# BarisYazici/deep-rl-grasping

Measured on NVIDIA H100. Metric: SAC grad-steps/sec (batch 256, 64x64 depth), higher is better.
Workload: dtype bf16x3 (fp32-faithful split, f32 accumulate)

## Files before the change

### deep-rl-grasping_b200/csrc/common.cuh

```cuda
#pragma once
#include <cuda_runtime.h>
#include <stdint.h>

#include <string>
#include <vector>

namespace b2g {

#ifdef __CUDACC__
__device__ __forceinline__ void pdl_wait() { asm volatile("griddepcontrol.wait;" ::: "memory"); }
__device__ __forceinline__ void pdl_trigger() { asm volatile("griddepcontrol.launch_dependents;" ::: "memory"); }
template <typename... KArgs, typename... Args>
inline cudaError_t launch_pdl(void (*kernel)(KArgs...), dim3 grid, dim3 block, size_t smem, cudaStream_t s, bool pdl, Args... args) {
  cudaLaunchConfig_t cfg{};
  cfg.gridDim = grid; cfg.blockDim = block; cfg.dynamicSmemBytes = smem; cfg.stream = s;
  cudaLaunchAttribute attr[1];
  attr[0].id = cudaLaunchAttributeProgrammaticStreamSerialization;
  attr[0].val.programmaticStreamSerializationAllowed = 1;
  cfg.attrs = attr; cfg.numAttrs = pdl ? 1 : 0;
  return cudaLaunchKernelEx(&cfg, kernel, KArgs(args)...);
}
#endif
bool pdl_enabled();

// ... 76 lines not shown
struct TailArgs {
  int B, H, A, feat_dim;
  float gamma, target_entropy;
  int grad_scale_B;
  const float* z0_pi; const float* z0_vf; const float* z0_q1; const float* z0_q2; const float* z0_vt;
  int z0v_ld;
  HeadW pi, vf, q1, q2, vt;
  const float* ksig; const float* bsig;
  HeadG g_pi, g_vf, g_q1, g_q2;
  float* g_ksig; float* g_bsig;
  const float* log_alpha; float* g_log_alpha;
  const float* act;  int act_stride;
  const float* eps;
  const float* rew; const float* done;
  float* a0_pi; float* a0_vf; float* a0_q1; float* a0_q2;
  float* dz1_pi; float* dz1_vf; float* dz1_q1; float* dz1_q2;
  float* dz0_pi;
  float* dz0_v3;
  uint16_t* dz0_pi_p[2]; uint16_t* dz0_v3_p[2];
  float* per_sample;
  float* pi_out;
  float* metrics;
};
cudaError_t tail_launch(const TailArgs& a, cudaStream_t s);

struct HeadsWgradArgs {
  const float* X0[4];
  const float* dz0[4];
  const float* a0[4];
  const float* dz1[4];
  float* g_k0[4]; float* g_b0[4]; float* g_k1[4]; float* g_b1[4];
  int M0[4];
  int dz0_ld[4];
  int x0_ld, B;
  int H;
};
void heads_wgrad_launch(const HeadsWgradArgs& a, cudaStream_t s);
cudaError_t act_launch(const TailArgs& t, int n, int deterministic, float* act_out, cudaStream_t s);

enum Metric : int {
  MET_POLICY_LOSS = 0, MET_QF1_LOSS, MET_QF2_LOSS, MET_VALUE_LOSS, MET_ENT_COEF_LOSS, MET_ENTROPY,
  MET_MEAN_Q1, MET_MEAN_Q2, MET_MEAN_V, MET_MEAN_LOGP, MET_GN_PI, MET_GN_VALUES, MET_COUNT = 16
};

struct OptimArgs {
  float* P; float* Mo; float* Vo; const float* G;
  float* T;
// ... 129 lines not shown
```

### deep-rl-grasping_b200/csrc/engine_v2.cu

```cuda
#include <cuda_bf16.h>

#include <algorithm>
#include <cstdio>
#include <cstdlib>
#include <cstring>

#include "sac_internal.cuh"

namespace b2g {
namespace {

struct Gather2Args {
  GatherArgs g;
  uint16_t* s1[2][3];
  uint16_t* fp[3][3];
  int KF;
};

__device__ __forceinline__ void split3(float y, uint16_t& p0, uint16_t& p1, uint16_t& p2) {
  const __nv_bfloat16 h0 = __float2bfloat16_rn(y);
  const float r1 = y - __bfloat162float(h0);
  const __nv_bfloat16 h1 = __float2bfloat16_rn(r1);
  const float r2 = r1 - __bfloat162float(h1);
  p0 = __bfloat16_as_ushort(h0); p1 = __bfloat16_as_ushort(h1); p2 = __bfloat16_as_ushort(__float2bfloat16_rn(r2));
// ... 98 lines not shown
      split3(av, p0, p1, p2);
      const size_t po = (size_t)b * a.KF + feat_dim + tid;
      a.fp[1][0][po] = p0; a.fp[1][1][po] = p1; a.fp[1][2][po] = p2;
    }
    if (tid == 32) {
      float r = g.rew[slot];
      if (g.normc[4] != 0.0) r = (float)fmin(fmax((double)r * g.normc[0], -g.normc[2]), g.normc[2]);
      g.rew_out[b] = r;
      g.done_out[b] = g.done[slot];
    }
  }
}

struct Plane2Job {
  const float* src;
  uint16_t* dst[3];
  int R, N, np;
  int transpose;
  int ld, off0;
  int k1_ci;
  int tile_start;
};

__global__ void __launch_bounds__(256) planes2_kernel(const Plane2Job* __restrict__ jobs, const int* __restrict__ cta_job) {
  __shared__ float tile[64][33];
  const Plane2Job job = jobs[cta_job[blockIdx.x]];
  const int t = blockIdx.x - job.tile_start;
  const int tiles_n = (job.N + 31) / 32;
  const int r0 = (t / tiles_n) * 64, n0 = (t % tiles_n) * 32;
  const int tid = threadIdx.x;
  const bool vec_ok = (job.N & 3) == 0;
  for (int i = tid; i < 64 * 8; i += 256) {
    const int rr = i >> 3, c4 = i & 7, r = r0 + rr, n = n0 + 4 * c4;
    float4 v = make_float4(0.f, 0.f, 0.f, 0.f);
    if (r < job.R) {
      const float* sp = job.src + (size_t)r * job.N + n;
      if (vec_ok && n + 3 < job.N) v = *reinterpret_cast<const float4*>(sp);
      else { if (n < job.N) v.x = sp[0]; if (n + 1 < job.N) v.y = sp[1]; if (n + 2 < job.N) v.z = sp[2]; if (n + 3 < job.N) v.w = sp[3]; }
    }
    tile[rr][4 * c4] = v.x; tile[rr][4 * c4 + 1] = v.y; tile[rr][4 * c4 + 2] = v.z; tile[rr][4 * c4 + 3] = v.w;
    if (!job.transpose && r < job.R) {
      const float x[4] = {v.x, v.y, v.z, v.w};
      uint16_t p[3][4];
#pragma unroll
      for (int u = 0; u < 4; ++u) split3(x[u], p[0][u], p[1][u], p[2][u]);
      for (int k = 0; k < job.np; ++k) {
        uint16_t* d = job.dst[k] + (size_t)r * job.ld + job.off0 + n;
        if (n + 3 < job.N && (((size_t)r * job.ld + job.off0 + n) & 3) == 0)
          *reinterpret_cast<uint2*>(d) = make_uint2((uint32_t)p[k][0] | ((uint32_t)p[k][1] << 16), (uint32_t)p[k][2] | ((uint32_t)p[k][3] << 16));
        else
          for (int u = 0; u < 4; ++u) if (n + u < job.N) d[u] = p[k][u];
      }
    }
  }
  if (!job.transpose) return;
  __syncthreads();
  {
    const int nn = tid >> 3, g8 = tid & 7, n = n0 + nn, rb = r0 + 8 * g8;
    if (n < job.N && rb < job.R) {
      uint16_t p[3][8];
#pragma unroll
      for (int u = 0; u < 8; ++u) split3(tile[8 * g8 + u][nn], p[0][u], p[1][u], p[2][u]);
      const size_t o = (size_t)(n + job.off0) * job.ld + rb;
      for (int k = 0; k < job.np; ++k) {
        uint16_t* d = job.dst[k] + o;
        if (job.k1_ci) {
          for (int u = 0; u < 8; ++u) if (rb + u < job.R) d[conv1_krow(rb + u, job.k1_ci) - rb] = p[k][u];
        } else if (rb + 7 < job.R && (o & 7) == 0)
          *reinterpret_cast<uint4*>(d) = make_uint4((uint32_t)p[k][0] | ((uint32_t)p[k][1] << 16), (uint32_t)p[k][2] | ((uint32_t)p[k][3] << 16),
                                                    (uint32_t)p[k][4] | ((uint32_t)p[k][5] << 16), (uint32_t)p[k][6] | ((uint32_t)p[k][7] << 16));
        else
          for (int u = 0; u < 8; ++u) if (rb + u < job.R) d[u] = p[k][u];
      }
    }
  }
}

int add_maps(V2State& v, uint16_t* const* planes, int np, int rank, std::initializer_list<uint64_t> dims, std::initializer_list<uint64_t> strides_b,
             std::initializer_list<uint32_t> box, std::initializer_list<uint32_t> estr = {}, bool allow_whole = true, int swizzle = 128) {
  uint64_t d[5] = {1, 1, 1, 1, 1}, s[5] = {0, 0, 0, 0, 0};
  uint32_t bx[5] = {1, 1, 1, 1, 1}, es[5] = {1, 1, 1, 1, 1};
  int i = 0; for (auto x : dims) d[i++] = x;
  i = 0; for (auto x : strides_b) s[i++] = x;
  i = 0; for (auto x : box) bx[i++] = x;
  i = 0; for (auto x : estr) es[i++] = x;
  if (rank >= 5 || np < 1) return -1;
  size_t rows = 1;
// ... 175 lines not shown
  if (int rc = palloc(v.W1T[0], 3, (size_t)64 * K1)) return rc;
  if (int rc = palloc(v.W1T[1], 3, (size_t)32 * K1)) return rc;
  for (int n = 0; n < 3; ++n) {
    if (int rc = palloc(v.W2T[n], 3, 64 * 512)) return rc;
    if (int rc = palloc(v.W3T[n], 3, 64 * 576)) return rc;
    if (int rc = palloc(v.WfT[n], 3, 512 * 1024)) return rc;
    if (int rc = palloc(v.K0T[n], 3, (size_t)(n == 1 ? 3 : 1) * h->H * KF)) return rc;
  }
  return 0;
}

int v2_create(b2g_sac* h) {
  V2State& v = h->v2;
  g_mk_state = &v;
  const int B = h->B, Ci = h->Cimg, Cp = s2d_channels(Ci), K1 = 64 * Cp, KF = v.KF, FS = h->FS, H = h->H;
  const size_t n1 = (size_t)B * 225 * 32;
  const char* nets[3] = {"model/pi", "model/values_fn", "target/values_fn"};
  std::vector<Plane2Job> jobs;
  int start = 0;
  auto add_job = [&](const float* src, int R, int N, uint16_t* const* dst, int np, int transpose, int ld, int off0) {
    Plane2Job j{};
    j.src = src; j.R = R; j.N = N; j.np = np; j.transpose = transpose; j.ld = ld; j.off0 = off0; j.tile_start = start;
    for (int k = 0; k < np; ++k) j.dst[k] = dst[k];
    start += ((R + 63) / 64) * ((N + 31) / 32);
    jobs.push_back(j);
  };
  add_job(h->p("model/pi/cnn1/w"), 64 * Ci, 32, v.W1T[0], 3, 1, K1, 0);
  jobs.back().k1_ci = Ci;
  add_job(h->p("model/values_fn/cnn1/w"), 64 * Ci, 32, v.W1T[0], 3, 1, K1, 32);
  jobs.back().k1_ci = Ci;
  add_job(h->p("target/values_fn/cnn1/w"), 64 * Ci, 32, v.W1T[1], 3, 1, K1, 0);
  jobs.back().k1_ci = Ci;
  for (int n = 0; n < 3; ++n) {
    add_job(h->p(std::string(nets[n]) + "/cnn2/w"), 512, 64, v.W2T[n], 3, 1, 512, 0);
    add_job(h->p(std::string(nets[n]) + "/cnn3/w"), 576, 64, v.W3T[n], 3, 1, 576, 0);
    add_job(h->p(std::string(nets[n]) + "/cnn_fc1/w"), 1024, 512, v.WfT[n], 3, 1, 1024, 0);
  }
  add_job(h->p("model/pi/fc0/kernel"), h->feat_dim, H, v.K0T[0], 3, 1, KF, 0);
  add_job(h->p("model/values_fn/vf/fc0/kernel"), h->feat_dim, H, v.K0T[1], 3, 1, KF, 0);
  add_job(h->p("model/values_fn/qf1/fc0/kernel"), h->feat_dim + h->A, H, v.K0T[1], 3, 1, KF, H);
  add_job(h->p("model/values_fn/qf2/fc0/kernel"), h->feat_dim + h->A, H, v.K0T[1], 3, 1, KF, 2 * H);
  add_job(h->p("target/values_fn/vf/fc0/kernel"), h->feat_dim, H, v.K0T[2], 3, 1, KF, 0);
  for (int n = 0; n < 2; ++n) {
    add_job(h->p(std::string(nets[n]) + "/cnn2/w"), 512, 64, v.W2n[n], 2, 0, 64, 0);
    add_job(h->p(std::string(nets[n]) + "/cnn3/w"), 576, 64, v.W3n[n], 2, 0, 64, 0);
    add_job(h->p(std::string(nets[n]) + "/cnn_fc1/w"), 1024, 512, v.Wfn[n], 2, 0, 512, 0);
  }
  add_job(h->p("model/pi/fc0/kernel"), h->feat_dim, H, v.K0n[0], 2, 0, H, 0);
  add_job(h->p("model/values_fn/vf/fc0/kernel"), h->feat_dim, H, v.K0n[1], 2, 0, 3 * H, 0);
  add_job(h->p("model/values_fn/qf1/fc0/kernel"), h->feat_dim + h->A, H, v.K0n[1], 2, 0, 3 * H, H);
  add_job(h->p("model/values_fn/qf2/fc0/kernel"), h->feat_dim + h->A, H, v.K0n[1], 2, 0, 3 * H, 2 * H);
  v.n_plane_jobs = (int)jobs.size();
  v.plane_ctas = start;
  Plane2Job* dj = nullptr;
  if (int rc = dev_alloc(h->allocs, h->stream, &dj, jobs.size())) return rc;
  CK(cudaMemcpyAsync(dj, jobs.data(), jobs.size() * sizeof(Plane2Job), cudaMemcpyHostToDevice, h->stream));
  CK(cudaStreamSynchronize(h->stream));
  v.plane_jobs = dj;
  {
    std::vector<int> cj((size_t)start);
    for (size_t k = 0; k < jobs.size(); ++k)
      for (int t = jobs[k].tile_start; t < (k + 1 < jobs.size() ? jobs[k + 1].tile_start : start); ++t) cj[t] = (int)k;
    if (int rc = upload_table(h->allocs, h->stream, cj, &v.plane_cta_job)) return rc;
  }

// ... 355 lines not shown
    std::vector<const CgGroup*> pa(parts.begin(), parts.begin() + 2), pb(parts.begin() + 2, parts.end());
    std::vector<Wire> wa, wb;
    for (int n = 0; n < 2; ++n) {
      wa.push_back({1, 2 * n, 0, n, 128, 128, 0});
      wa.push_back({1, 2 * n + 1, 0, n, 64, 128, 1});
      wb.push_back({1, n, 0, 2 * n, 72, 108, 0});
      wb.push_back({2, n, 0, 2 * n, 144, 108, 1});
    }
    wb.push_back({2, 2, 1, 0, 1, 8, 1});
    wb.push_back({2, 2, 1, 1, 1, 8, 1});
    if (int rc = fuse_groups(h, pa, wa, "bwd_fused_fc", v.bwd_fused, n_ctr)) return rc;
    if (int rc = fuse_groups(h, pb, wb, "bwd_fused_conv", v.bwd_fused, n_ctr)) return rc;
  }
  if (int rc = dev_alloc(h->allocs, h->stream, &v.dep_ctr, (size_t)n_ctr)) return rc;
  v.n_dep_ctr = n_ctr;
  bind_counters(v.fwd_fused, v.dep_ctr);
  bind_counters(v.bwd_fused, v.dep_ctr);
  if (int rc = dev_alloc(h->allocs, h->stream, &v.d_maps, v.maps.size())) return rc;
  CK(cudaMemcpyAsync(v.d_maps, v.maps.data(), v.maps.size() * sizeof(CUtensorMap), cudaMemcpyHostToDevice, h->stream));
  CK(cudaStreamSynchronize(h->stream));
  return 0;
}

int v2_planes(b2g_sac* h, cudaStream_t s) {
  V2State& v = h->v2;
  planes2_kernel<<<v.plane_ctas, 256, 0, s>>>((const Plane2Job*)v.plane_jobs, v.plane_cta_job);
  return 0;
}

int v2_gather(b2g_sac* h, const GatherArgs& ga, cudaStream_t s) {
  V2State& v = h->v2;
  Gather2Args a{};
  a.g = ga;
  for (int w = 0; w < 2; ++w)
    for (int p = 0; p < 3; ++p) a.s1[w][p] = v.S[w][p];
  for (int n = 0; n < 3; ++n) for (int p = 0; p < 3; ++p) a.fp[n][p] = v.F[n][p];
  a.KF = v.KF;
  const dim3 grid(ga.B, ga.next_obs || ga.next_frame ? 2 : 1);
  switch (h->Cimg) {
    case 1: gather2_kernel<1><<<grid, 512, 0, s>>>(a); break;
    case 2: gather2_kernel<2><<<grid, 512, 0, s>>>(a); break;
    case 3: gather2_kernel<3><<<grid, 512, 0, s>>>(a); break;
    default: gather2_kernel<4><<<grid, 512, 0, s>>>(a); break;
  }
  return 0;
}

extern long long* g_cg_trace;
static long long* s_trace_buf = nullptr;
// ... 38 lines not shown
```

### deep-rl-grasping_b200/csrc/sac.cu

```cuda
#include <cuda_runtime.h>
#include <math.h>
#include <stdio.h>
#include <string.h>

#include <algorithm>
#include <chrono>
#include <map>
#include <tuple>
#include <string>
#include <vector>

#include "../../include/b200grasp.h"
#include "common.cuh"
#include "sac_internal.cuh"
#include "state.cuh"

using namespace b2g;

namespace b2g {
bool pdl_enabled() {
  static int v = -1;
  if (v < 0) { const char* e = getenv("B2G_PDL"); v = (e && e[0] == '0') ? 0 : 1; }
  return v != 0;
}
// ... 602 lines not shown
  cudaStream_t s = h->stream;
  int n = 0;
  int n_copy = 0;
  (void)n_copy;
  auto mark = [&](const char* name) {
    if (prof && prof->on) {
      cudaEvent_t e;
      cudaEventCreate(&e);
      cudaEventRecord(e, s);
      prof->ev.push_back(e);
      prof->names.push_back(name);
    }
  };
  mark("begin");
  PrepArgs pa = make_prep(h, h->cfg.seed + 0x9E3779B97F4A7C15ull * (unsigned long long)h->cfg.rank, sampled, apply);
  const bool fork = h->fork_leaves && !(prof && prof->on);
  cudaStream_t ax = fork ? h->aux : s;
  GatherArgs ga = make_gather(h, sampled, true);
  if (fork) {
    pa.defer_bump = 1; pa.skip_indices = 1;
    if (sampled) { ga.indices = nullptr; ga.rng_counters = h->counters; ga.seed = pa.seed; ga.indices_out = h->indices; }
    CK(cudaEventRecord(h->ev_aux[0], s));
    CK(cudaStreamWaitEvent(ax, h->ev_aux[0], 0));
    if (h->use_planes && !h->v2.on) { planes_launch(h->d_jobs, h->n_jobs, h->job_tiles, ax); ++n; }
    if (h->v2.on) { if (int rc = v2_planes(h, ax)) return rc; ++n; }
    CK(cudaMemsetAsync(h->z0[0], 0, (size_t)5 * h->B * h->H * sizeof(float), ax)); ++n_copy;
    if (h->v2.on) { CK(cudaMemsetAsync(h->v2.z0v, 0, (size_t)3 * h->B * h->H * sizeof(float), ax)); ++n_copy; }
    CK(cudaEventRecord(h->ev_aux[1], ax));
    prep_launch(pa, ax); ++n;
    CK(cudaMemsetAsync(h->G, 0, (size_t)(h->n_train + MET_COUNT) * sizeof(float), ax)); ++n_copy;
    CK(cudaEventRecord(h->ev_aux[6], ax));
  } else {
    prep_launch(pa, s); ++n; mark("prep");
  }
  if (h->v2.on) {
    if (!fork) { if (int rc = v2_planes(h, s)) return rc; ++n; mark("weight_planes_v2"); }
    if (int rc = v2_gather(h, ga, s)) return rc;
  } else gather_launch(ga, s);
  ++n; mark("gather_normalize");
  if (h->record_after_gather) CK(cudaEventRecord(h->record_after_gather, s));
  if (fork) CK(cudaStreamWaitEvent(s, h->ev_aux[1], 0));
  else {
    CK(cudaMemsetAsync(h->G, 0, (size_t)(h->n_train + MET_COUNT) * sizeof(float), s)); ++n_copy;
    CK(cudaMemsetAsync(h->z0[0], 0, (size_t)5 * h->B * h->H * sizeof(float), s)); ++n_copy;
    if (h->v2.on) { CK(cudaMemsetAsync(h->v2.z0v, 0, (size_t)3 * h->B * h->H * sizeof(float), s)); ++n_copy; }
    mark("zero_grads");
  }
  const int x3 = h->cfg.precision == B2G_PREC_BF16X3 ? 1 : 0;
  auto run_group = [&](GemmGroup& g, cudaStream_t s) -> int {
    if (g.tc) CK(gg_tc_launch(g.host.data(), (int)g.host.size(), g.total_tiles, g.host[0].flags, x3, h->num_sms, s));
    else gg_simt_launch(g.dev, (int)g.host.size(), g.total_tiles, s);
    ++n; mark(g.name.c_str());
    return 0;
  };
  if (h->v2.on) {
    CK(cudaMemsetAsync(h->v2.dep_ctr, 0, (size_t)h->v2.n_dep_ctr * sizeof(int), s)); ++n_copy;
    if (int rc = v2_launch(h, h->v2.fwd_fused[0], s)) return rc;
    ++n; mark("fwd_fused");
  } else {
    for (auto& g : h->fwd_groups) if (int rc = run_group(g, s)) return rc;
  }
  if (fork) CK(cudaStreamWaitEvent(s, h->ev_aux[6], 0));
  CK(tail_launch(make_tail(h, want_per_sample), s)); ++n; mark("heads_tail");
  auto make_optim = [&]() {
    OptimArgs oa{};
    oa.P = h->P; oa.Mo = h->Mo; oa.Vo = h->Vo; oa.G = h->G; oa.T = h->P + h->n_train;
    oa.n_pi = (int)h->n_pi; oa.n_values = (int)h->n_values; oa.n_ent = (int)h->n_ent; oa.n_target = (int)h->n_target;
    oa.step_consts = h->step_consts; oa.tau = h->cfg.tau; oa.grad_scale = 1.0f / (float)h->cfg.nranks;
    oa.metrics = h->metrics; oa.apply = apply ? 1 : 0;
    return oa;
  };
  const bool overlap = h->overlap_ar && h->cfg.nranks > 1 && !(h->dp_p2p && apply);
  const int64_t pi_fc1 = h->tensors[h->tindex.at("model/pi/" + std::string(h->cnn ? "cnn_fc1/w" : "fc0/kernel"))].off;
  const int64_t v_fc1 = h->tensors[h->tindex.at("model/values_fn/" + std::string(h->cnn ? "cnn_fc1/w" : "vf/fc0/kernel"))].off;
  auto nccl_ck = [&](int rc) -> int {
    if (rc != 0) return b2g_fail(B2G_ENCCL, std::string("nccl: ") + (g_nccl.GetErrorString ? g_nccl.GetErrorString(rc) : "?"));
    return 0;
  };
  bool dp_early_opt = false;
  if (h->v2.on) {
    h->v2.sm_reserve = 0;
    cudaStream_t lx = fork ? ax : s;
    if (fork) { CK(cudaEventRecord(h->ev_aux[2], s)); CK(cudaStreamWaitEvent(ax, h->ev_aux[2], 0)); }
    HeadsWgradArgs wa{};
    const char* hp[4] = {"model/pi", "model/values_fn/vf", "model/values_fn/qf1", "model/values_fn/qf2"};
    for (int q = 0; q < 4; ++q) {
      wa.X0[q] = h->F[q == 0 ? 0 : 1];
      wa.dz0[q] = q == 0 ? h->dz0_pi : h->dz0_v3 + (q - 1) * h->H;
      wa.dz0_ld[q] = q == 0 ? h->H : 3 * h->H;
      wa.a0[q] = h->a0[q]; wa.dz1[q] = h->dz1[q];
      wa.M0[q] = q >= 2 ? h->feat_dim + h->A : h->feat_dim;
      wa.g_k0[q] = h->g(std::string(hp[q]) + "/fc0/kernel"); wa.g_b0[q] = h->g(std::string(hp[q]) + "/fc0/bias");
      wa.g_k1[q] = h->g(std::string(hp[q]) + "/fc1/kernel"); wa.g_b1[q] = h->g(std::string(hp[q]) + "/fc1/bias");
    }
    wa.x0_ld = h->FS; wa.B = h->B; wa.H = h->H;
    heads_wgrad_launch(wa, lx); ++n; if (!fork) mark("heads_wgrad");
    if (!overlap) {
      if (int rc = v2_launch(h, h->v2.bwd_fused[0], s)) return rc;
      ++n; mark("bwd_fused");
    } else {
      if (int rc = v2_launch(h, h->v2.bwd_fused[1], s)) return rc;
      ++n; mark("bwd_fused_fc");
      CK(cudaMemcpyAsync(h->G + h->n_train, h->metrics, MET_GN_PI * sizeof(float), cudaMemcpyDeviceToDevice, s)); ++n_copy;
      CK(cudaEventRecord(h->ev_fork, s));
      CK(cudaStreamWaitEvent(h->side, h->ev_fork, 0));
      if (fork) { CK(cudaEventRecord(h->ev_aux[4], ax)); CK(cudaStreamWaitEvent(h->side, h->ev_aux[4], 0)); }
// ... 307 lines not shown
          }
      };
      patch(h->v2.bwd_fused);
      if (found && (t.off & 3) == 0) { h->dp_skip[k][0] = (int)(t.off >> 2); h->dp_skip[k][1] = (int)((t.off + 1024 * 512) >> 2); }
    }
  }
  h->dp_p2p = true;
  if (h->graph_exec) { cudaGraphExecDestroy(h->graph_exec); h->graph_exec = nullptr; }
  for (auto& g : h->pipe_graph) if (g) { cudaGraphExecDestroy(g); g = nullptr; }
  return 0;
}

int b2g_sac_destroy(b2g_sac* h) {
  if (!h) return 0;
  cudaSetDevice(h->cfg.device);
  if (h->stream) cudaStreamSynchronize(h->stream);
  if (h->graph_exec) cudaGraphExecDestroy(h->graph_exec);
  for (auto& g : h->pipe_graph) if (g) cudaGraphExecDestroy(g);
  for (void* q : h->dp_opened) cudaIpcCloseMemHandle(q);
  nccl_comm_destroy(h->nccl_comm2);
  nccl_comm_destroy(h->nccl_comm);
  if (h->side) cudaStreamDestroy(h->side);
  if (h->aux) { cudaStreamSynchronize(h->aux); cudaStreamDestroy(h->aux); }
  for (auto& e : h->ev_aux) if (e) cudaEventDestroy(e);
  if (h->ev_fork) cudaEventDestroy(h->ev_fork);
  if (h->ev_join) cudaEventDestroy(h->ev_join);
  for (void* q : h->allocs) cudaFree(q);
  for (int q = 0; q < 2; ++q) { if (h->hc_obs[q]) cudaFreeHost(h->hc_obs[q]); if (h->hc_next[q]) cudaFreeHost(h->hc_next[q]); }
  if (h->h_met) cudaFreeHost(h->h_met);
  if (h->h_cnt) cudaFreeHost(h->h_cnt);
  if (h->h_plan) cudaFreeHost(h->h_plan);
  if (h->h_rc) cudaFreeHost(h->h_rc);
  for (int k = 0; k < 2; ++k) { if (h->hp_stats[k]) cudaFreeHost(h->hp_stats[k]); if (h->ev_stats[k]) cudaEventDestroy(h->ev_stats[k]); }
  for (int j = 0; j < 2; ++j) {
    if (h->ev_h2d[j]) cudaEventDestroy(h->ev_h2d[j]);
    if (h->ev_consumed[j]) cudaEventDestroy(h->ev_consumed[j]);
    if (h->ev_met[j]) cudaEventDestroy(h->ev_met[j]);
    if (h->pm_met[j]) cudaFreeHost(h->pm_met[j]);
    if (h->pm_cnt[j]) cudaFreeHost(h->pm_cnt[j]);
  }
  if (h->cstream) cudaStreamDestroy(h->cstream);
  if (h->ev0) cudaEventDestroy(h->ev0);
  if (h->ev1) cudaEventDestroy(h->ev1);
  if (h->stream) cudaStreamDestroy(h->stream);
  delete h;
  return 0;
// ... 134 lines not shown
  DA(h->z0[0], 5 * B * h->H);
  for (int q = 1; q < 5; ++q) h->z0[q] = h->z0[0] + (size_t)q * B * h->H;
  for (int q = 0; q < 4; ++q) { DA(h->a0[q], B * h->H); DA(h->dz1[q], B * h->H); }
  DA(h->dz0_pi, B * h->H); DA(h->dz0_v3, B * 3 * h->H);
  DA(h->per_sample, 7 * B); DA(h->pi_out, B * h->A); DA(h->eps, B * h->A + 4); DA(h->rew_n, B); DA(h->done_n, B);
  DA(h->indices, B + 4);
#undef DA
  if (cudaMallocHost((void**)&h->h_met, (MET_COUNT + 2) * sizeof(float)) != cudaSuccess ||
      cudaMallocHost((void**)&h->h_cnt, 8 * sizeof(long long)) != cudaSuccess)
    return bail(b2g_fail(B2G_ECUDA, "cudaMallocHost failed"));
  for (int j = 0; j < 2; ++j) {
    if ((rc = dev_alloc(h->allocs, h->stream, &h->ps_obs[j], (size_t)B * h->Ec)) || (rc = dev_alloc(h->allocs, h->stream, &h->ps_next[j], (size_t)B * h->Ec))) return bail(rc);
    if (cudaEventCreateWithFlags(&h->ev_h2d[j], cudaEventDisableTiming) != cudaSuccess ||
        cudaEventCreateWithFlags(&h->ev_consumed[j], cudaEventDisableTiming) != cudaSuccess ||
        cudaEventCreateWithFlags(&h->ev_met[j], cudaEventDisableTiming) != cudaSuccess ||
        cudaMallocHost((void**)&h->pm_met[j], (MET_COUNT + 2) * sizeof(float)) != cudaSuccess ||
        cudaMallocHost((void**)&h->pm_cnt[j], 8 * sizeof(long long)) != cudaSuccess)
      return bail(b2g_fail(B2G_ECUDA, "pipelined-path resources"));
  }
  if (cudaStreamCreateWithFlags(&h->cstream, cudaStreamNonBlocking) != cudaSuccess) return bail(b2g_fail(B2G_ECUDA, "copy stream"));
  {
    const char* fk = getenv("B2G_FORK");
    if (!(fk && atoi(fk) == 0)) {
      if (cudaStreamCreateWithFlags(&h->aux, cudaStreamNonBlocking) != cudaSuccess) return bail(b2g_fail(B2G_ECUDA, "aux stream"));
      for (auto& e : h->ev_aux)
        if (cudaEventCreateWithFlags(&e, cudaEventDisableTiming) != cudaSuccess) return bail(b2g_fail(B2G_ECUDA, "aux events"));
      h->fork_leaves = true;
    }
  }
  {
    std::vector<double> ones(h->Ec, 1.0);
    if (cudaMemcpyAsync(h->d_istd, ones.data(), h->Ec * sizeof(double), cudaMemcpyHostToDevice, h->stream) != cudaSuccess ||
        cudaStreamSynchronize(h->stream) != cudaSuccess)
      return bail(b2g_fail(B2G_ECUDA, "init copy failed"));
  }
  if ((rc = build_groups(h))) return bail(rc);
  if (h->v2.on && (rc = v2_create(h))) return bail(rc);
  if (cfg->nranks > 1) {
    if (!cfg->nccl_id) return bail(b2g_fail(B2G_EINVAL, "nranks > 1 needs nccl_id"));
    if ((rc = nccl_comm_init(&h->nccl_comm, cfg->nranks, cfg->nccl_id, cfg->rank, cfg->nccl_lib))) return bail(rc);
    {
      const char* ov = getenv("B2G_AR_OVERLAP");
      const bool want_ov = h->v2.on && !(ov && ov[0] == '0');
      if (want_ov && g_nccl.CommSplit && g_nccl.GroupStart && g_nccl.GroupEnd) {
        if (g_nccl.CommSplit(h->nccl_comm, 0, cfg->rank, &h->nccl_comm2, nullptr) == 0 && h->nccl_comm2 &&
            cudaStreamCreateWithFlags(&h->side, cudaStreamNonBlocking) == cudaSuccess &&
            cudaEventCreateWithFlags(&h->ev_fork, cudaEventDisableTiming) == cudaSuccess &&
// ... 535 lines not shown
  s[4].pieces = {dev_piece(h->r_nfr, cap * sizeof(int))};
  s[5].pieces = {dev_piece(h->r_act, cap * h->A * sizeof(float))};
  s[6].pieces = {dev_piece(h->r_rew, cap * sizeof(float))};
  s[7].pieces = {dev_piece(h->r_done, cap * sizeof(float))};
  s[8].pieces = frame_pieces(h, lo, hi);
  for (int i = 0; i < 9; ++i) s[i].tag = kSacTags[i + 2];
  return s;
}

}

extern "C" {

int b2g_sac_state_save(b2g_sac* h, const char* path) {
  if (!h || !path) return b2g_fail(B2G_EINVAL, "NULL argument");
  B2G_USABLE(h);
  if (h->cfg.nranks > 1)
    return b2g_fail(B2G_ESTATE, "training-state files of data-parallel learners (nranks > 1) are not built: each rank holds only its "
                                "slice of the Adam moments");
  if (h->pipe_pending)
    return b2g_fail(B2G_ESTATE, "a host-pipelined step is in flight: call b2g_sac_pipeline_flush first (its losses would be lost)");
  CK(cudaSetDevice(h->cfg.device));
  CK(cudaStreamSynchronize(h->stream));
  if (h->aux) CK(cudaStreamSynchronize(h->aux));
  long long cnt[8];
  CK(cudaMemcpy(cnt, h->counters, sizeof cnt, cudaMemcpyDeviceToHost));
  SacHostState hs;
  hs.r_size = h->r_size; hs.head_seq = h->head_seq; hs.tail_seq = h->tail_seq; hs.next_fid = h->next_fid; hs.evicted = h->evicted;
  hs.lw.assign(h->lw.begin(), h->lw.end());
  hs.prev_next = h->prev_next;
  std::vector<int64_t> hv = {hs.r_size, hs.head_seq, hs.tail_seq, hs.next_fid, hs.evicted, (int64_t)hs.lw.size(), (int64_t)hs.prev_next.size()};
  for (const auto& q : hs.lw) { hv.push_back(q.first); hv.push_back(q.second); }
  hv.insert(hv.end(), hs.prev_next.begin(), hs.prev_next.end());
  std::vector<StateSection> secs(2);
  secs[0].tag = kSacTags[0]; secs[0].pieces = {host_piece(hv.data(), hv.size() * sizeof(int64_t))};
  secs[1].tag = kSacTags[1]; secs[1].pieces = {host_piece(cnt, sizeof cnt)};
  for (auto& s : sac_device_sections(h, hs.frame_lo(h->frame_cap), hs.next_fid)) secs.push_back(std::move(s));
  if (h->rms_mean) {
    StateSection r;
    r.tag = kRmsTag;
    r.pieces = {host_piece(&h->rms_count, sizeof(double)), dev_piece(h->rms_mean, h->E * sizeof(double)),
                dev_piece(h->rms_var, h->E * sizeof(double))};
    secs.push_back(std::move(r));
  }
  return state_write(path, STATE_KIND_SAC, sac_fingerprint_rms(h), secs);
}

// ... 24 lines not shown
  const int64_t cap = h->cfg.buffer_capacity, FC = h->frame_cap;
  if (rd.bytes(0) % 8 || rd.bytes(0) < 7 * 8 || rd.bytes(0) > (uint64_t)(7 + 2 * cap + 4 * FC) * 8)
    return b2g_fail(B2G_EINVAL, "corrupt replay bookkeeping in the training-state file");
  std::vector<int64_t> hv(rd.bytes(0) / 8);
  if (int rc = rd.read_host(0, hv.data(), hv.size() * 8)) return rc;
  SacHostState hs;
  hs.r_size = hv[0]; hs.head_seq = hv[1]; hs.tail_seq = hv[2]; hs.next_fid = hv[3]; hs.evicted = hv[4];
  const int64_t n_lw = hv[5], n_prev = hv[6];
  if (n_lw < 0 || n_prev < 0 || (int64_t)hv.size() != 7 + 2 * n_lw + n_prev || hs.r_size != hs.head_seq - hs.tail_seq || hs.r_size < 0 ||
      hs.r_size > cap || hs.tail_seq < 0 || hs.next_fid < 0 || hs.evicted < 0)
    return b2g_fail(B2G_EINVAL, "corrupt replay bookkeeping in the training-state file");
  for (int64_t i = 0; i < n_lw; ++i) hs.lw.emplace_back(hv[7 + 2 * i], hv[8 + 2 * i]);
  hs.prev_next.assign(hv.begin() + 7 + 2 * n_lw, hv.end());
  const int64_t lo = hs.frame_lo(FC);
  if (lo < 0 || lo > hs.next_fid || hs.next_fid - lo > FC) return b2g_fail(B2G_EINVAL, "corrupt replay bookkeeping in the training-state file");
  std::vector<StateSection> dev = sac_device_sections(h, lo, hs.next_fid);
  for (int i = 0; i < (int)dev.size(); ++i)
    if (rd.bytes(i + 2) != dev[i].bytes())
      return b2g_fail(B2G_EINVAL, "training-state section lengths do not match this handle's configuration");
  long long cnt[8];
  if (rd.bytes(1) != sizeof cnt) return b2g_fail(B2G_EINVAL, "training-state section lengths do not match this handle's configuration");
  if (int rc = rd.read_host(1, cnt, sizeof cnt)) return rc;
  CK(cudaStreamSynchronize(h->stream));
  if (h->aux) CK(cudaStreamSynchronize(h->aux));
  h->broken = true;
  for (int i = 0; i < (int)dev.size(); ++i)
    if (int rc = rd.read_pieces(i + 2, dev[i].pieces)) return rc;
  if (h->rms_mean) {
    double count = 0.0;
    if (int rc = rd.read_pieces(n_sec, {host_piece(&count, sizeof(double)), dev_piece(h->rms_mean, h->E * sizeof(double)),
                                        dev_piece(h->rms_var, h->E * sizeof(double))})) return rc;
    h->rms_count = count;
    obs_rms_derive(h);
  }
  h->ob_n = 0;
  CK(cudaMemcpy(h->counters, cnt, sizeof cnt, cudaMemcpyHostToDevice));
  h->r_size = hs.r_size; h->head_seq = hs.head_seq; h->tail_seq = hs.tail_seq; h->next_fid = hs.next_fid; h->evicted = hs.evicted;
  h->lw.assign(hs.lw.begin(), hs.lw.end());
  h->prev_next = hs.prev_next;
  h->planes_dirty = true;
  h->broken = false;
  return 0;
}

}
```

### deep-rl-grasping_b200/csrc/sac_internal.cuh

```cuda
#pragma once
#include <cuda_runtime.h>

#include <deque>
#include <map>
#include <string>
#include <tuple>
#include <vector>

#include "../../include/b200grasp.h"
#include "cg.cuh"
#include "common.cuh"
#include "host.cuh"

namespace b2g {
struct Tensor {
  std::string name;
  int ndim;
  int64_t shape[4];
  int64_t numel;
  int64_t off;
  int group;
};


// ... 7 lines not shown
  int KF = 576;
  uint16_t* S[2][3]{};
  uint16_t* H1[3][3]{};
  uint16_t* H2[3][3]{};
  uint16_t* H3[3][3]{};
  uint16_t* F[3][3]{};
  uint16_t* dz0pi[2]{};
  uint16_t* dz0v[2]{};
  uint16_t* dZ4[2][2]{};
  uint16_t* dZ3[2][2]{};
  uint16_t* dZ2[2][2]{};
  uint16_t* dZ1[2]{};
  uint16_t* W1T[2][3]{};
  uint16_t* W2T[3][3]{};
  uint16_t* W3T[3][3]{};
  uint16_t* WfT[3][3]{};
  uint16_t* K0T[3][3]{};
  uint16_t* W2n[2][2]{};
  uint16_t* W3n[2][2]{};
  uint16_t* Wfn[2][2]{};
  uint16_t* K0n[2][2]{};
  float* z0v = nullptr;
  void* plane_jobs = nullptr; int n_plane_jobs = 0, plane_ctas = 0;
  const int* plane_cta_job = nullptr;
  int sm_reserve = 0;
  std::vector<CUtensorMap> maps;
  std::vector<char> map_whole;
  std::vector<int> map_box_bytes;
  CUtensorMap* d_maps = nullptr;
  std::vector<CgGroup> fwd, bwd_groups;
  std::vector<CgGroup> fwd_fused, bwd_fused;
  int split_fc1 = 3;
  int split_fc1_dgrad = 1;
  int* dep_ctr = nullptr; int n_dep_ctr = 0;
  std::vector<int*> tabs;
  int dbg = 0;
};

}

struct b2g_sac;
namespace b2g {
int v2_alloc(b2g_sac* h);
int v2_create(b2g_sac* h);
int v2_planes(b2g_sac* h, cudaStream_t s);
int v2_gather(b2g_sac* h, const GatherArgs& ga, cudaStream_t s);
int v2_launch(b2g_sac* h, const CgGroup& g, cudaStream_t s);
int sac_act_rows(b2g_sac* h, const float* rows, int chunk, int deterministic);
int sac_replay_add_linked(b2g_sac* h, const float* c_obs, const float* c_next, const int64_t* obs_fid, const float* act,
                          const float* rew, const float* done, int n, int64_t* next_fid);
void obs_rms_derive(b2g_sac* h);
}

using namespace b2g;

struct b2g_sac {
  b2g_sac_cfg cfg{};
  bool cnn = false;
  int num_sms = 132;
  int B = 0, A = 0, H = 0, E = 0, Cimg = 0, feat_dim = 0, FS = 0;
  int Hi = 0, Wi = 0, H1 = 0, W1 = 0, H2 = 0, W2 = 0, H3 = 0, W3 = 0;
  std::vector<Tensor> tensors;
  std::map<std::string, int> tindex;
  int64_t n_pi = 0, n_values = 0, n_ent = 0, n_target = 0, n_train = 0, n_all = 0;
  float *P = nullptr, *Mo = nullptr, *Vo = nullptr, *G = nullptr;
  float* metrics = nullptr;
  cudaStream_t stream = nullptr;
  std::vector<void*> allocs;
// ... 43 lines not shown
  long long* pm_cnt[2]{};
  long long pipe_k = 0;
  bool pipe_pending = false;
  cudaEvent_t record_after_gather = nullptr;
  long long* counters = nullptr;
  double* step_consts = nullptr;
  float* d_lr = nullptr;
  float cur_lr = -1.f;
  std::vector<GemmGroup> fwd_groups, bwd_groups, act_groups;
  cudaGraphExec_t graph_exec = nullptr;
  bool use_graph = true;
  void* nccl_comm = nullptr;
  void* nccl_comm2 = nullptr;
  bool pipe_serial = false; int pipe_tune = 0; double pipe_t0 = 0, pipe_period[2] = {0, 0};
  bool dp_p2p = false;
  int* dp_x = nullptr;
  int* dp_sync = nullptr;
  float* dp_recv = nullptr;
  float* dp_P[8]{}; float* dp_G[8]{}; int* dp_X[8]{};
  std::vector<void*> dp_opened;
  int dp_skip[2][2]{};
  cudaStream_t side = nullptr;
  cudaStream_t aux = nullptr;
  cudaEvent_t ev_aux[7]{};
  bool fork_leaves = false;
  std::map<std::tuple<const void*, const void*, const void*, int>, int> col_ids;
  cudaEvent_t ev_fork = nullptr, ev_join = nullptr;
  bool overlap_ar = false;
  int ar_sms = 8;
  ColsumJob* d_colsum_early = nullptr;
  int n_colsum_early = 0, colsum_early_ctas = 0;
  cudaEvent_t ev0 = nullptr, ev1 = nullptr;
  float last_ms = 0.f;
  int launches = 0;
  std::vector<std::string> prof_names;
  float* h_met = nullptr;
  long long* h_cnt = nullptr;

  b2g::V2State v2;
  bool broken = false;
  double* hp_stats[2]{};
  cudaEvent_t ev_stats[2]{};
  int stats_k = 0;
  double norm_eps = 1e-8;

  double *rms_mean = nullptr, *rms_var = nullptr;
  double rms_count = 0.0;
// ... 13 lines not shown
```

### deep-rl-grasping_b200/csrc/tail.cu

```cuda
#include <math.h>

#include <cuda_bf16.h>

#include "common.cuh"

namespace b2g {
namespace {
constexpr int H = 64, LD = 65, WARPS = 8, AMAX = 8;
constexpr float EPSF = 1e-6f, LS_MAX = 2.0f, LS_MIN = -20.0f;

struct V2 { float lo, hi; };

__device__ __forceinline__ float warp_sum(float v) {
#pragma unroll
  for (int o = 16; o > 0; o >>= 1) v += __shfl_xor_sync(0xffffffffu, v, o);
  return v;
}
__device__ __forceinline__ V2 relu2(V2 a) { return V2{fmaxf(a.lo, 0.f), fmaxf(a.hi, 0.f)}; }

__device__ __forceinline__ V2 fwd64(const float* __restrict__ Ws, const float* __restrict__ bias, V2 a, int lane) {
  V2 o{bias[lane], bias[lane + 32]};
#pragma unroll 8
  for (int i = 0; i < 32; ++i) {
    const float ai = __shfl_sync(0xffffffffu, a.lo, i);
// ... 731 lines not shown
      if (!deterministic) u += t.eps[b * A + a] * expf(fminf(fmaxf(sc[g * 2 * AMAX + AMAX + a], LS_MIN), LS_MAX));
      act_out[b * A + a] = tanhf(u);
    }
  }
}

template <int H>
size_t tailw_smem() { return sizeof(float) * tw_smem_floats<H>(); }
template <int H>
size_t actw_smem() { return sizeof(float) * (2 * (size_t)TW_KS * (H + 1) + 2 * TW_G * H + TW_G * 2 * AMAX); }

template <class K>
cudaError_t smem_optin(K* fn, size_t bytes, unsigned long long& done) {
  int dev = 0;
  if (cudaError_t e = cudaGetDevice(&dev)) return e;
  const unsigned long long bit = dev < 64 ? 1ull << dev : 0ull;
  if (done & bit) return cudaSuccess;
  if (cudaError_t e = cudaFuncSetAttribute(fn, cudaFuncAttributeMaxDynamicSharedMemorySize, (int)bytes)) return e;
  done |= bit;
  return cudaSuccess;
}

template <int H>
cudaError_t tailw_launch(const TailArgs& a, cudaStream_t s) {
  static unsigned long long done = 0;
  if (cudaError_t e = smem_optin(tailw_kernel<H>, tailw_smem<H>(), done)) return e;
  return launch_pdl(tailw_kernel<H>, dim3((a.B + TW_G - 1) / TW_G), dim3(H), tailw_smem<H>(), s, pdl_enabled(), a);
}
template <int H>
cudaError_t actw_launch(const TailArgs& t, int n, int deterministic, float* act_out, cudaStream_t s) {
  static unsigned long long done = 0;
  if (cudaError_t e = smem_optin(actw_kernel<H>, actw_smem<H>(), done)) return e;
  actw_kernel<H><<<(n + TW_G - 1) / TW_G, H, actw_smem<H>(), s>>>(t, n, deterministic, act_out);
  return cudaPeekAtLastError();
}

}

cudaError_t act_launch(const TailArgs& t, int n, int deterministic, float* act_out, cudaStream_t s) {
  if (n <= 0) return cudaSuccess;
  switch (t.H) {
    case 128: return actw_launch<128>(t, n, deterministic, act_out, s);
    case 192: return actw_launch<192>(t, n, deterministic, act_out, s);
    case 256: return actw_launch<256>(t, n, deterministic, act_out, s);
  }
  act_kernel<<<(n + WARPS - 1) / WARPS, WARPS * 32, 0, s>>>(t, n, deterministic, act_out);
  return cudaPeekAtLastError();
}

namespace {
// ... 37 lines not shown
  float* __restrict__ G = (fc1 ? a.g_k1[q] : a.g_k0[q]) + n0;
#pragma unroll
  for (int i = 0; i < 4; ++i) {
    const int r = row0 + 4 * ty + i;
    if (r < M)
      asm volatile("red.global.add.v4.f32 [%0], {%1,%2,%3,%4};" ::"l"(G + (size_t)r * H + 4 * tx), "f"(acc[i][0]), "f"(acc[i][1]), "f"(acc[i][2]),
                   "f"(acc[i][3])
                   : "memory");
  }
  if (sums && tid < 64) atomicAdd((fc1 ? a.g_b1[q] : a.g_b0[q]) + n0 + tid, cs);
}
}

void heads_wgrad_launch(const HeadsWgradArgs& a, cudaStream_t s) {
  heads_wgrad_kernel<<<dim3(9 + a.H / 64, 4, HW_KSPLIT * (a.H / 64)), 256, 0, s>>>(a);
}

static size_t tail_smem(int A) {
  return sizeof(float) * (S_NW * H * LD + 2 * H * A + 2 * A + 3 * (H + 1) + MET_COUNT + 1 + 8 +
                           (S_NW * 2 * H + 2 * H * A + 2 * A + 4 * (H + 1) + 2 * A * H + 8) +
                           64);
}

cudaError_t tail_launch(const TailArgs& a, cudaStream_t s) {
  switch (a.H) {
    case 128: return tailw_launch<128>(a, s);
    case 192: return tailw_launch<192>(a, s);
    case 256: return tailw_launch<256>(a, s);
  }
  static unsigned long long done = 0;
  if (cudaError_t e = smem_optin(tail4_kernel, tail_smem(AMAX), done)) return e;
  const int grid = (a.B + 1) / 2;
  return launch_pdl(tail4_kernel, dim3(grid), dim3(WARPS * 32), tail_smem(a.A), s, pdl_enabled(), a);
}

}
```

Measured before the change: 2443.

## Split weight-plane conversion into fwd/bwd halves and overlap across extra aux stream

Result: faster. 2565 (median of 6 runs) (+5.0%).

```diff
diff --git a/deep-rl-grasping_b200/csrc/common.cuh b/deep-rl-grasping_b200/csrc/common.cuh
--- a/deep-rl-grasping_b200/csrc/common.cuh
+++ b/deep-rl-grasping_b200/csrc/common.cuh
@@ -122,7 +122,7 @@
   float* pi_out;
   float* metrics;
 };
-cudaError_t tail_launch(const TailArgs& a, cudaStream_t s);
+cudaError_t tail_launch(const TailArgs& a, cudaStream_t s, bool pdl);
 
 struct HeadsWgradArgs {
   const float* X0[4];
diff --git a/deep-rl-grasping_b200/csrc/engine_v2.cu b/deep-rl-grasping_b200/csrc/engine_v2.cu
--- a/deep-rl-grasping_b200/csrc/engine_v2.cu
+++ b/deep-rl-grasping_b200/csrc/engine_v2.cu
@@ -144,47 +144,66 @@
   int tile_start;
 };
 
-__global__ void __launch_bounds__(256) planes2_kernel(const Plane2Job* __restrict__ jobs, const int* __restrict__ cta_job) {
-  __shared__ float tile[64][33];
-  const Plane2Job job = jobs[cta_job[blockIdx.x]];
-  const int t = blockIdx.x - job.tile_start;
-  const int tiles_n = (job.N + 31) / 32;
-  const int r0 = (t / tiles_n) * 64, n0 = (t % tiles_n) * 32;
+constexpr int P2_SUB = 4;
+__global__ void __launch_bounds__(256) planes2_kernel(const Plane2Job* __restrict__ jobs, const int* __restrict__ cta_job, int cta0) {
+  __shared__ float tile[P2_SUB][64][33];
+  const int cta = cta0 + blockIdx.x;
+  const Plane2Job job = jobs[cta_job[cta]];
+  const int t = cta - job.tile_start;
+  const int strips_n = (job.N + 32 * P2_SUB - 1) / (32 * P2_SUB);
+  const int r0 = (t / strips_n) * 64, nb = (t % strips_n) * 32 * P2_SUB;
   const int tid = threadIdx.x;
   const bool vec_ok = (job.N & 3) == 0;
-  for (int i = tid; i < 64 * 8; i += 256) {
-    const int rr = i >> 3, c4 = i & 7, r = r0 + rr, n = n0 + 4 * c4;
-    float4 v = make_float4(0.f, 0.f, 0.f, 0.f);
-    if (r < job.R) {
-      const float* sp = job.src + (size_t)r * job.N + n;
-      if (vec_ok && n + 3 < job.N) v = *reinterpret_cast<const float4*>(sp);
-      else { if (n < job.N) v.x = sp[0]; if (n + 1 < job.N) v.y = sp[1]; if (n + 2 < job.N) v.z = sp[2]; if (n + 3 < job.N) v.w = sp[3]; }
-    }
-    tile[rr][4 * c4] = v.x; tile[rr][4 * c4 + 1] = v.y; tile[rr][4 * c4 + 2] = v.z; tile[rr][4 * c4 + 3] = v.w;
-    if (!job.transpose && r < job.R) {
-      const float x[4] = {v.x, v.y, v.z, v.w};
-      uint16_t p[3][4];
-#pragma unroll
-      for (int u = 0; u < 4; ++u) split3(x[u], p[0][u], p[1][u], p[2][u]);
-      for (int k = 0; k < job.np; ++k) {
-        uint16_t* d = job.dst[k] + (size_t)r * job.ld + job.off0 + n;
-        if (n + 3 < job.N && (((size_t)r * job.ld + job.off0 + n) & 3) == 0)
-          *reinterpret_cast<uint2*>(d) = make_uint2((uint32_t)p[k][0] | ((uint32_t)p[k][1] << 16), (uint32_t)p[k][2] | ((uint32_t)p[k][3] << 16));
-        else
-          for (int u = 0; u < 4; ++u) if (n + u < job.N) d[u] = p[k][u];
-      }
-    }
-  }
+  float4 v[P2_SUB][2];
+#pragma unroll
+  for (int q = 0; q < P2_SUB; ++q)
+#pragma unroll
+    for (int j = 0; j < 2; ++j) {
+      const int i = tid + 256 * j, r = r0 + (i >> 3), n = nb + 32 * q + 4 * (i & 7);
+      v[q][j] = make_float4(0.f, 0.f, 0.f, 0.f);
+      if (r < job.R && n < job.N) {
+        const float* sp = job.src + (size_t)r * job.N + n;
+        if (vec_ok && n + 3 < job.N) v[q][j] = *reinterpret_cast<const float4*>(sp);
+        else { v[q][j].x = sp[0]; if (n + 1 < job.N) v[q][j].y = sp[1]; if (n + 2 < job.N) v[q][j].z = sp[2]; if (n + 3 < job.N) v[q][j].w = sp[3]; }
+      }
+    }
+#pragma unroll
+  for (int q = 0; q < P2_SUB; ++q)
+#pragma unroll
+    for (int j = 0; j < 2; ++j) {
+      const int i = tid + 256 * j, rr = i >> 3, c4 = i & 7, r = r0 + rr, n = nb + 32 * q + 4 * c4;
+      if (job.transpose) {
+        tile[q][rr][4 * c4] = v[q][j].x; tile[q][rr][4 * c4 + 1] = v[q][j].y; tile[q][rr][4 * c4 + 2] = v[q][j].z; tile[q][rr][4 * c4 + 3] = v[q][j].w;
+      } else if (r < job.R && n < job.N) {
+        const float x[4] = {v[q][j].x, v[q][j].y, v[q][j].z, v[q][j].w};
+        uint16_t p[3][4];
+#pragma unroll
+        for (int u = 0; u < 4; ++u) split3(x[u], p[0][u], p[1][u], p[2][u]);
+#pragma unroll
+        for (int k = 0; k < 3; ++k) {
+          if (k == job.np) break;
+          uint16_t* d = job.dst[k] + (size_t)r * job.ld + job.off0 + n;
+          if (n + 3 < job.N && (((size_t)r * job.ld + job.off0 + n) & 3) == 0)
+            *reinterpret_cast<uint2*>(d) = make_uint2((uint32_t)p[k][0] | ((uint32_t)p[k][1] << 16), (uint32_t)p[k][2] | ((uint32_t)p[k][3] << 16));
+          else
+            for (int u = 0; u < 4; ++u) if (n + u < job.N) d[u] = p[k][u];
+        }
+      }
+    }
   if (!job.transpose) return;
   __syncthreads();
-  {
-    const int nn = tid >> 3, g8 = tid & 7, n = n0 + nn, rb = r0 + 8 * g8;
+  const int nn = tid >> 3, g8 = tid & 7, rb = r0 + 8 * g8;
+#pragma unroll
+  for (int q = 0; q < P2_SUB; ++q) {
+    const int n = nb + 32 * q + nn;
     if (n < job.N && rb < job.R) {
       uint16_t p[3][8];
 #pragma unroll
-      for (int u = 0; u < 8; ++u) split3(tile[8 * g8 + u][nn], p[0][u], p[1][u], p[2][u]);
+      for (int u = 0; u < 8; ++u) split3(tile[q][8 * g8 + u][nn], p[0][u], p[1][u], p[2][u]);
       const size_t o = (size_t)(n + job.off0) * job.ld + rb;
-      for (int k = 0; k < job.np; ++k) {
+#pragma unroll
+      for (int k = 0; k < 3; ++k) {
+        if (k == job.np) break;
         uint16_t* d = job.dst[k] + o;
         if (job.k1_ci) {
           for (int u = 0; u < 8; ++u) if (rb + u < job.R) d[conv1_krow(rb + u, job.k1_ci) - rb] = p[k][u];
@@ -406,7 +425,7 @@
     Plane2Job j{};
     j.src = src; j.R = R; j.N = N; j.np = np; j.transpose = transpose; j.ld = ld; j.off0 = off0; j.tile_start = start;
     for (int k = 0; k < np; ++k) j.dst[k] = dst[k];
-    start += ((R + 63) / 64) * ((N + 31) / 32);
+    start += ((R + 63) / 64) * ((N + 32 * P2_SUB - 1) / (32 * P2_SUB));
     jobs.push_back(j);
   };
   add_job(h->p("model/pi/cnn1/w"), 64 * Ci, 32, v.W1T[0], 3, 1, K1, 0);
@@ -425,6 +444,7 @@
   add_job(h->p("model/values_fn/qf1/fc0/kernel"), h->feat_dim + h->A, H, v.K0T[1], 3, 1, KF, H);
   add_job(h->p("model/values_fn/qf2/fc0/kernel"), h->feat_dim + h->A, H, v.K0T[1], 3, 1, KF, 2 * H);
   add_job(h->p("target/values_fn/vf/fc0/kernel"), h->feat_dim, H, v.K0T[2], 3, 1, KF, 0);
+  v.plane_ctas_fwd = start;
   for (int n = 0; n < 2; ++n) {
     add_job(h->p(std::string(nets[n]) + "/cnn2/w"), 512, 64, v.W2n[n], 2, 0, 64, 0);
     add_job(h->p(std::string(nets[n]) + "/cnn3/w"), 576, 64, v.W3n[n], 2, 0, 64, 0);
@@ -826,9 +846,10 @@
   return 0;
 }
 
-int v2_planes(b2g_sac* h, cudaStream_t s) {
+int v2_planes(b2g_sac* h, bool backward, cudaStream_t s) {
   V2State& v = h->v2;
-  planes2_kernel<<<v.plane_ctas, 256, 0, s>>>((const Plane2Job*)v.plane_jobs, v.plane_cta_job);
+  const int cta0 = backward ? v.plane_ctas_fwd : 0, n = backward ? v.plane_ctas - v.plane_ctas_fwd : v.plane_ctas_fwd;
+  planes2_kernel<<<n, 256, 0, s>>>((const Plane2Job*)v.plane_jobs, v.plane_cta_job, cta0);
   return 0;
 }
 
diff --git a/deep-rl-grasping_b200/csrc/sac.cu b/deep-rl-grasping_b200/csrc/sac.cu
--- a/deep-rl-grasping_b200/csrc/sac.cu
+++ b/deep-rl-grasping_b200/csrc/sac.cu
@@ -648,24 +648,33 @@
     if (sampled) { ga.indices = nullptr; ga.rng_counters = h->counters; ga.seed = pa.seed; ga.indices_out = h->indices; }
     CK(cudaEventRecord(h->ev_aux[0], s));
     CK(cudaStreamWaitEvent(ax, h->ev_aux[0], 0));
+    CK(cudaStreamWaitEvent(h->aux2, h->ev_aux[0], 0));
     if (h->use_planes && !h->v2.on) { planes_launch(h->d_jobs, h->n_jobs, h->job_tiles, ax); ++n; }
-    if (h->v2.on) { if (int rc = v2_planes(h, ax)) return rc; ++n; }
+    if (h->v2.on) { if (int rc = v2_planes(h, false, ax)) return rc; ++n; }
     CK(cudaMemsetAsync(h->z0[0], 0, (size_t)5 * h->B * h->H * sizeof(float), ax)); ++n_copy;
-    if (h->v2.on) { CK(cudaMemsetAsync(h->v2.z0v, 0, (size_t)3 * h->B * h->H * sizeof(float), ax)); ++n_copy; }
+    if (h->v2.on) {
+      CK(cudaMemsetAsync(h->v2.z0v, 0, (size_t)3 * h->B * h->H * sizeof(float), ax)); ++n_copy;
+      CK(cudaMemsetAsync(h->v2.dep_ctr, 0, (size_t)h->v2.n_dep_ctr * sizeof(int), ax)); ++n_copy;
+    }
     CK(cudaEventRecord(h->ev_aux[1], ax));
-    prep_launch(pa, ax); ++n;
-    CK(cudaMemsetAsync(h->G, 0, (size_t)(h->n_train + MET_COUNT) * sizeof(float), ax)); ++n_copy;
-    CK(cudaEventRecord(h->ev_aux[6], ax));
+    prep_launch(pa, h->aux2); ++n;
+    CK(cudaMemsetAsync(h->G, 0, (size_t)(h->n_train + MET_COUNT) * sizeof(float), h->aux2)); ++n_copy;
+    CK(cudaEventRecord(h->ev_aux[6], h->aux2));
   } else {
     prep_launch(pa, s); ++n; mark("prep");
   }
   if (h->v2.on) {
-    if (!fork) { if (int rc = v2_planes(h, s)) return rc; ++n; mark("weight_planes_v2"); }
+    if (!fork) {
+      if (int rc = v2_planes(h, false, s)) return rc;
+      ++n; mark("weight_planes_fwd");
+      if (int rc = v2_planes(h, true, s)) return rc;
+      ++n; mark("weight_planes_bwd");
+    }
     if (int rc = v2_gather(h, ga, s)) return rc;
   } else gather_launch(ga, s);
   ++n; mark("gather_normalize");
   if (h->record_after_gather) CK(cudaEventRecord(h->record_after_gather, s));
-  if (fork) CK(cudaStreamWaitEvent(s, h->ev_aux[1], 0));
+  if (fork) { CK(cudaStreamWaitEvent(s, h->ev_aux[1], 0)); CK(cudaStreamWaitEvent(s, h->ev_aux[6], 0)); }
   else {
     CK(cudaMemsetAsync(h->G, 0, (size_t)(h->n_train + MET_COUNT) * sizeof(float), s)); ++n_copy;
     CK(cudaMemsetAsync(h->z0[0], 0, (size_t)5 * h->B * h->H * sizeof(float), s)); ++n_copy;
@@ -680,14 +689,19 @@
     return 0;
   };
   if (h->v2.on) {
-    CK(cudaMemsetAsync(h->v2.dep_ctr, 0, (size_t)h->v2.n_dep_ctr * sizeof(int), s)); ++n_copy;
+    if (!fork) { CK(cudaMemsetAsync(h->v2.dep_ctr, 0, (size_t)h->v2.n_dep_ctr * sizeof(int), s)); ++n_copy; }
     if (int rc = v2_launch(h, h->v2.fwd_fused[0], s)) return rc;
     ++n; mark("fwd_fused");
   } else {
     for (auto& g : h->fwd_groups) if (int rc = run_group(g, s)) return rc;
   }
-  if (fork) CK(cudaStreamWaitEvent(s, h->ev_aux[6], 0));
-  CK(tail_launch(make_tail(h, want_per_sample), s)); ++n; mark("heads_tail");
+  if (fork && h->v2.on) {
+    CK(cudaEventRecord(h->ev_aux[7], s)); CK(cudaStreamWaitEvent(ax, h->ev_aux[7], 0));
+    if (int rc = v2_planes(h, true, ax)) return rc;
+    ++n;
+    CK(cudaEventRecord(h->ev_aux[8], ax));
+  }
+  CK(tail_launch(make_tail(h, want_per_sample), s, pdl_enabled() && !h->v2.on)); ++n; mark("heads_tail");
   auto make_optim = [&]() {
     OptimArgs oa{};
     oa.P = h->P; oa.Mo = h->Mo; oa.Vo = h->Vo; oa.G = h->G; oa.T = h->P + h->n_train;
@@ -707,7 +721,10 @@
   if (h->v2.on) {
     h->v2.sm_reserve = 0;
     cudaStream_t lx = fork ? ax : s;
-    if (fork) { CK(cudaEventRecord(h->ev_aux[2], s)); CK(cudaStreamWaitEvent(ax, h->ev_aux[2], 0)); }
+    if (fork) {
+      CK(cudaStreamWaitEvent(s, h->ev_aux[8], 0));
+      CK(cudaEventRecord(h->ev_aux[2], s)); CK(cudaStreamWaitEvent(ax, h->ev_aux[2], 0));
+    }
     HeadsWgradArgs wa{};
     const char* hp[4] = {"model/pi", "model/values_fn/vf", "model/values_fn/qf1", "model/values_fn/qf2"};
     for (int q = 0; q < 4; ++q) {
@@ -1061,6 +1078,7 @@
   nccl_comm_destroy(h->nccl_comm);
   if (h->side) cudaStreamDestroy(h->side);
   if (h->aux) { cudaStreamSynchronize(h->aux); cudaStreamDestroy(h->aux); }
+  if (h->aux2) { cudaStreamSynchronize(h->aux2); cudaStreamDestroy(h->aux2); }
   for (auto& e : h->ev_aux) if (e) cudaEventDestroy(e);
   if (h->ev_fork) cudaEventDestroy(h->ev_fork);
   if (h->ev_join) cudaEventDestroy(h->ev_join);
@@ -1241,7 +1259,8 @@
   {
     const char* fk = getenv("B2G_FORK");
     if (!(fk && atoi(fk) == 0)) {
-      if (cudaStreamCreateWithFlags(&h->aux, cudaStreamNonBlocking) != cudaSuccess) return bail(b2g_fail(B2G_ECUDA, "aux stream"));
+      if (cudaStreamCreateWithFlags(&h->aux, cudaStreamNonBlocking) != cudaSuccess ||
+          cudaStreamCreateWithFlags(&h->aux2, cudaStreamNonBlocking) != cudaSuccess) return bail(b2g_fail(B2G_ECUDA, "aux stream"));
       for (auto& e : h->ev_aux)
         if (cudaEventCreateWithFlags(&e, cudaEventDisableTiming) != cudaSuccess) return bail(b2g_fail(B2G_ECUDA, "aux events"));
       h->fork_leaves = true;
@@ -1823,7 +1842,7 @@
     return b2g_fail(B2G_ESTATE, "a host-pipelined step is in flight: call b2g_sac_pipeline_flush first (its losses would be lost)");
   CK(cudaSetDevice(h->cfg.device));
   CK(cudaStreamSynchronize(h->stream));
-  if (h->aux) CK(cudaStreamSynchronize(h->aux));
+  if (h->aux) { CK(cudaStreamSynchronize(h->aux)); CK(cudaStreamSynchronize(h->aux2)); }
   long long cnt[8];
   CK(cudaMemcpy(cnt, h->counters, sizeof cnt, cudaMemcpyDeviceToHost));
   SacHostState hs;
@@ -1894,7 +1913,7 @@
   if (rd.bytes(1) != sizeof cnt) return b2g_fail(B2G_EINVAL, "training-state section lengths do not match this handle's configuration");
   if (int rc = rd.read_host(1, cnt, sizeof cnt)) return rc;
   CK(cudaStreamSynchronize(h->stream));
-  if (h->aux) CK(cudaStreamSynchronize(h->aux));
+  if (h->aux) { CK(cudaStreamSynchronize(h->aux)); CK(cudaStreamSynchronize(h->aux2)); }
   h->broken = true;
   for (int i = 0; i < (int)dev.size(); ++i)
     if (int rc = rd.read_pieces(i + 2, dev[i].pieces)) return rc;
diff --git a/deep-rl-grasping_b200/csrc/sac_internal.cuh b/deep-rl-grasping_b200/csrc/sac_internal.cuh
--- a/deep-rl-grasping_b200/csrc/sac_internal.cuh
+++ b/deep-rl-grasping_b200/csrc/sac_internal.cuh
@@ -53,6 +53,7 @@
   uint16_t* K0n[2][2]{};
   float* z0v = nullptr;
   void* plane_jobs = nullptr; int n_plane_jobs = 0, plane_ctas = 0;
+  int plane_ctas_fwd = 0;
   const int* plane_cta_job = nullptr;
   int sm_reserve = 0;
   std::vector<CUtensorMap> maps;
@@ -74,7 +75,7 @@
 namespace b2g {
 int v2_alloc(b2g_sac* h);
 int v2_create(b2g_sac* h);
-int v2_planes(b2g_sac* h, cudaStream_t s);
+int v2_planes(b2g_sac* h, bool backward, cudaStream_t s);
 int v2_gather(b2g_sac* h, const GatherArgs& ga, cudaStream_t s);
 int v2_launch(b2g_sac* h, const CgGroup& g, cudaStream_t s);
 int sac_act_rows(b2g_sac* h, const float* rows, int chunk, int deterministic);
@@ -164,7 +165,8 @@
   int dp_skip[2][2]{};
   cudaStream_t side = nullptr;
   cudaStream_t aux = nullptr;
-  cudaEvent_t ev_aux[7]{};
+  cudaStream_t aux2 = nullptr;
+  cudaEvent_t ev_aux[9]{};
   bool fork_leaves = false;
   std::map<std::tuple<const void*, const void*, const void*, int>, int> col_ids;
   cudaEvent_t ev_fork = nullptr, ev_join = nullptr;
diff --git a/deep-rl-grasping_b200/csrc/tail.cu b/deep-rl-grasping_b200/csrc/tail.cu
--- a/deep-rl-grasping_b200/csrc/tail.cu
+++ b/deep-rl-grasping_b200/csrc/tail.cu
@@ -777,10 +777,10 @@
 }
 
 template <int H>
-cudaError_t tailw_launch(const TailArgs& a, cudaStream_t s) {
+cudaError_t tailw_launch(const TailArgs& a, cudaStream_t s, bool pdl) {
   static unsigned long long done = 0;
   if (cudaError_t e = smem_optin(tailw_kernel<H>, tailw_smem<H>(), done)) return e;
-  return launch_pdl(tailw_kernel<H>, dim3((a.B + TW_G - 1) / TW_G), dim3(H), tailw_smem<H>(), s, pdl_enabled(), a);
+  return launch_pdl(tailw_kernel<H>, dim3((a.B + TW_G - 1) / TW_G), dim3(H), tailw_smem<H>(), s, pdl, a);
 }
 template <int H>
 cudaError_t actw_launch(const TailArgs& t, int n, int deterministic, float* act_out, cudaStream_t s) {
@@ -864,16 +864,16 @@
                            64);
 }
 
-cudaError_t tail_launch(const TailArgs& a, cudaStream_t s) {
+cudaError_t tail_launch(const TailArgs& a, cudaStream_t s, bool pdl) {
   switch (a.H) {
-    case 128: return tailw_launch<128>(a, s);
-    case 192: return tailw_launch<192>(a, s);
-    case 256: return tailw_launch<256>(a, s);
+    case 128: return tailw_launch<128>(a, s, pdl);
+    case 192: return tailw_launch<192>(a, s, pdl);
+    case 256: return tailw_launch<256>(a, s, pdl);
   }
   static unsigned long long done = 0;
   if (cudaError_t e = smem_optin(tail4_kernel, tail_smem(AMAX), done)) return e;
   const int grid = (a.B + 1) / 2;
-  return launch_pdl(tail4_kernel, dim3(grid), dim3(WARPS * 32), tail_smem(a.A), s, pdl_enabled(), a);
-}
-
-}
+  return launch_pdl(tail4_kernel, dim3(grid), dim3(WARPS * 32), tail_smem(a.A), s, pdl, a);
+}
+
+}
```
